# KeyuWu-CS/MonoHair

Hardware: AMD Instinct MI355X
Metric: PMVO iterations/sec (60x1080p views, 256^3 volume) (higher is better)
Workload: dtype f32

## Files before the change

### monohair_amd/csrc/pmvo_search.hip

```cpp
#include "mh_search_common.h"
#include "../../include/mh_pmvo_lab.h"

__device__ __forceinline__ void mh_sample_next(const float *__restrict__ cam, float X0, float X1, float X2,
                                               float ori_r, float ori_c, float Hf, float Wf, float off, float &S0,
                                               float &S1, float &S2, int forms) {
    alignas(16) float rec[16];
    mh_sample_rank(cam, X0, X1, X2, ori_r, ori_c, Hf, Wf, rec, forms);
    mh_sample_item(reinterpret_cast<const float4 *>(rec), off, S0, S1, S2);
}

__device__ __forceinline__ float mh_one_minus_abs(float x) {
    float r;
    asm("v_sub_f32_e64 %0, 1.0, |%1|" : "=v"(r) : "v"(x));
    return r;
}

template <int K, int T>
__global__ __launch_bounds__(T) void mh_search_kernel(MhViews vw, const float *__restrict__ offs, int S, int nrank,
                                                      int rank_step, const float *__restrict__ pts, int N, int P1,
                                                      float thr, const float *__restrict__ ori_c,
                                                      const int32_t *__restrict__ base_idx,
                                                      const float *__restrict__ base_val,
                                                      const float4 *__restrict__ taps, float *__restrict__ line_ori,
                                                      float *__restrict__ min_loss, uint8_t *__restrict__ high_conf,
                                                      float *__restrict__ best_sample, int32_t *__restrict__ best_rank,
                                                      int32_t *__restrict__ best_s, MhRule rule) {
    __shared__ float s_loss[MH_MAX_ITEMS];
    __shared__ uint8_t s_pos[MH_MAX_ITEMS];
    __shared__ float s_rl[MH_MAX_RANKS];
    __shared__ int s_ri[MH_MAX_RANKS];
    __shared__ int s_rh[MH_MAX_RANKS];

    const int n = blockIdx.x, tid = threadIdx.x;
    const int nitems = nrank * S;
    const int V = vw.V;
    const float Hf = (float)vw.H, Wf = (float)vw.W;
    const float P0 = pts[3 * n], P1x = pts[3 * n + 1], P2 = pts[3 * n + 2];

    float X0[K], X1[K], X2[K];
    MhCascV num[K], den[K];
    int cnt[K];
    const int tail_from = mh_tail_from(rule, n, S);
#pragma unroll
    for (int j = 0; j < K; ++j) {
        int it = j * T + tid;
        it = it < nitems ? it : 0;
        const int r = it / S, s = it - r * S;
        const int b = min(max(base_idx[(size_t)(r * rank_step) * N + n], 0), V - 1);
        const float2 oc = reinterpret_cast<const float2 *>(ori_c)[(size_t)b * N + n];
        mh_sample_next(vw.cams + b * MH_CAM_STRIDE, P0, P1x, P2, oc.x, oc.y, Hf, Wf, offs[s], X0[j], X1[j], X2[j],
                       mh_group_forms(rule, r, V, b, S));
        num[j] = den[j] = MhCascV{0.0f, 0.0f, 0.0f};
        cnt[j] = 0;
    }

    for (int v = 0; v < V; ++v) {
        if (v > 0 && (v & 15) == 0) {
#pragma unroll
            for (int j = 0; j < K; ++j) {
                mh_cascv_flush(num[j], v);
                mh_cascv_flush(den[j], v);
            }
        }
        const float4 *__restrict__ rec = taps + ((size_t)v * N + n) * P1;
        const float4 hdr = rec[0];
        if (hdr.y == -1.0f) continue;
        const int ntap = __float_as_int(hdr.x);
        const float *__restrict__ cam = vw.cams + v * MH_CAM_STRIDE;
        const float4 t0 = rec[1];
        {
            float dx[K], dy[K], ml[K], bc[K];
#pragma unroll
            for (int j = 0; j < K; ++j) {
                float row, col;
                mh_pixel_of(cam, X0[j], X1[j], X2[j], Hf, Wf, row, col);
                mh_unit2(row - hdr.z, col - hdr.w, dx[j], dy[j]);
                const float cs = t0.x * dx[j] + t0.y * dy[j];
                ml[j] = 1.0f - __builtin_fabsf(cs);
                bc[j] = t0.z;
            }
            for (int t = 1; t < ntap; ++t) {
                const float4 tp = rec[1 + t];
#pragma unroll
                for (int j = 0; j < K; ++j) {
                    const float cs = tp.x * dx[j] + tp.y * dy[j];
                    const float l = 1.0f - __builtin_fabsf(cs);
                    const bool upd = l < ml[j];
                    ml[j] = upd ? l : ml[j];
                    bc[j] = upd ? tp.z : bc[j];
                }
            }
#pragma unroll
            for (int j = 0; j < K; ++j) {
                const float w = bc[j];
                num[j].a0 = num[j].a0 + ml[j] * w;
                den[j].a0 = den[j].a0 + w;
                cnt[j] += (w > 0.0f) ? 1 : 0;
            }
        }
    }

#pragma unroll
    for (int j = 0; j < K; ++j) {
        const int it = j * T + tid;
        if (it < nitems) {
            float dn = mh_cascv_done(den[j]);
            float nm = mh_cascv_done(num[j]);
            int cn = cnt[j];
            if (it - (it / S) * S >= tail_from)
                mh_tail_item_sums(vw.cams, V, Hf, Wf, taps + (size_t)n * P1, (size_t)N * P1, nullptr, N, X0[j], X1[j], X2[j],
                                  nm, dn, cn);
            const float ratio = dn / (float)cn;
            s_pos[it] = (ratio > thr) ? 1 : 0;
            s_loss[it] = nm / dn;
        }
    }
    const bool all_nan = mh_point_pixel_not_finite(vw, P0, P1x, P2, N, tid, T);

    const int wave = tid >> 6, lane = tid & 63, nwaves = T >> 6;
    for (int r = wave; r < nrank; r += nwaves) {
        int npos = 0;
        for (int s0 = 0; s0 < S; s0 += MH_WAVE) {
            const int s = s0 + lane;
            npos += __popcll(__ballot(s < S && s_pos[r * S + s]));
        }
        const bool low = npos < 5;
        float bl = 0.0f;
        int bi = 0x7fffffff;
        for (int s = lane; s < S; s += MH_WAVE) {
            float l = all_nan ? __builtin_nanf("") : s_loss[r * S + s];
            if (!low && !s_pos[r * S + s]) l = 1.0f;
            if (bi == 0x7fffffff || mh_min_better(l, s, bl, bi)) {
                bl = l;
                bi = s;
            }
        }
#pragma unroll
        for (int o = 32; o > 0; o >>= 1) {
            const float ol = __shfl_xor(bl, o);
            const int oi = __shfl_xor(bi, o);
            if (oi != 0x7fffffff && (bi == 0x7fffffff || mh_min_better(ol, oi, bl, bi))) {
                bl = ol;
                bi = oi;
            }
        }
        if (lane == 0) {
            s_rl[r] = bl;
            s_ri[r] = bi;
            s_rh[r] = s_pos[r * S + bi];
        }
    }
    __syncthreads();

    if (tid == 0) {
        const float Hf = (float)vw.H, Wf = (float)vw.W;
        float ml = s_rl[0];
        int br = 0, bs = s_ri[0], hc = s_rh[0];
        for (int r = 1; r < nrank; ++r) {
            const float l = s_rl[r];
            if ((l < ml) && (base_val[(size_t)(r * rank_step) * N + n] > 0.0f)) {
                ml = l;
                br = r;
                bs = s_ri[r];
                hc = s_rh[r];
            }
        }
        const int b = min(max(base_idx[(size_t)(br * rank_step) * N + n], 0), V - 1);
        const float2 oc = reinterpret_cast<const float2 *>(ori_c)[(size_t)b * N + n];
        float B0, B1, B2;
        mh_sample_next(vw.cams + b * MH_CAM_STRIDE, P0, P1x, P2, oc.x, oc.y, Hf, Wf, offs[bs], B0, B1, B2,
                       mh_group_forms(rule, br, V, b, S));
        const float d0 = B0 - P0, d1 = B1 - P1x, d2 = B2 - P2;
        float s2 = d0 * d0;
        s2 = mh_fma(d1, d1, s2);
        s2 = mh_fma(d2, d2, s2);
        const float nrm = __builtin_sqrtf(s2);
        line_ori[3 * n] = d0 / nrm;
        line_ori[3 * n + 1] = d1 / nrm;
        line_ori[3 * n + 2] = d2 / nrm;
        min_loss[n] = ml;
        high_conf[n] = (uint8_t)hc;
        if (best_sample) {
            best_sample[3 * n] = B0;
            best_sample[3 * n + 1] = B1;
            best_sample[3 * n + 2] = B2;
        }
        if (best_rank) best_rank[n] = br;
        if (best_s) best_s[n] = bs;
    }
}

__device__ __forceinline__ float mh_vmul(float a, float b) {
    float r;
    asm("v_mul_f32_e32 %0, %1, %2" : "=v"(r) : "v"(a), "v"(b));
    return r;
}
__device__ __forceinline__ float mh_vadd(float a, float b) {
    float r;
    asm("v_add_f32_e32 %0, %1, %2" : "=v"(r) : "v"(a), "v"(b));
    return r;
}

template <int KA>
__device__ __forceinline__ void mh_tap_update(float (&ML)[KA], float (&BC)[KA], const float (&l)[KA], float cf) {
    if constexpr (KA == 4) {
        unsigned long long m0, m1, m2, m3;
        asm("v_cmp_lt_f32_e64 %[m0], %[l0], %[a0]\n\t"
            "v_cmp_lt_f32_e64 %[m1], %[l1], %[a1]\n\t"
            "v_cmp_lt_f32_e64 %[m2], %[l2], %[a2]\n\t"
            "v_cmp_lt_f32_e64 %[m3], %[l3], %[a3]\n\t"
            "v_cndmask_b32_e64 %[a0], %[a0], %[l0], %[m0]\n\t"
            "v_cndmask_b32_e64 %[a1], %[a1], %[l1], %[m1]\n\t"
            "v_cndmask_b32_e64 %[a2], %[a2], %[l2], %[m2]\n\t"
            "v_cndmask_b32_e64 %[a3], %[a3], %[l3], %[m3]\n\t"
            "v_cndmask_b32_e64 %[b0], %[b0], %[cf], %[m0]\n\t"
            "v_cndmask_b32_e64 %[b1], %[b1], %[cf], %[m1]\n\t"
            "v_cndmask_b32_e64 %[b2], %[b2], %[cf], %[m2]\n\t"
            "v_cndmask_b32_e64 %[b3], %[b3], %[cf], %[m3]"
            : [a0] "+v"(ML[0]), [a1] "+v"(ML[1]), [a2] "+v"(ML[2]), [a3] "+v"(ML[3]), [b0] "+v"(BC[0]),
              [b1] "+v"(BC[1]), [b2] "+v"(BC[2]), [b3] "+v"(BC[3]), [m0] "=&s"(m0), [m1] "=&s"(m1), [m2] "=&s"(m2),
              [m3] "=&s"(m3)
            : [l0] "v"(l[0]), [l1] "v"(l[1]), [l2] "v"(l[2]), [l3] "v"(l[3]), [cf] "v"(cf));
    } else if constexpr (KA == 3) {
        unsigned long long m0, m1, m2;
        asm("v_cmp_lt_f32_e64 %[m0], %[l0], %[a0]\n\t"
            "v_cmp_lt_f32_e64 %[m1], %[l1], %[a1]\n\t"
            "v_cmp_lt_f32_e64 %[m2], %[l2], %[a2]\n\t"
            "v_cndmask_b32_e64 %[a0], %[a0], %[l0], %[m0]\n\t"
            "v_cndmask_b32_e64 %[a1], %[a1], %[l1], %[m1]\n\t"
            "v_cndmask_b32_e64 %[a2], %[a2], %[l2], %[m2]\n\t"
            "v_cndmask_b32_e64 %[b0], %[b0], %[cf], %[m0]\n\t"
            "v_cndmask_b32_e64 %[b1], %[b1], %[cf], %[m1]\n\t"
            "v_cndmask_b32_e64 %[b2], %[b2], %[cf], %[m2]"
            : [a0] "+v"(ML[0]), [a1] "+v"(ML[1]), [a2] "+v"(ML[2]), [b0] "+v"(BC[0]), [b1] "+v"(BC[1]),
              [b2] "+v"(BC[2]), [m0] "=&s"(m0), [m1] "=&s"(m1), [m2] "=&s"(m2)
            : [l0] "v"(l[0]), [l1] "v"(l[1]), [l2] "v"(l[2]), [cf] "v"(cf));
    } else if constexpr (KA == 2) {
        unsigned long long m0, m1;
        asm("v_cmp_lt_f32_e64 %[m0], %[l0], %[a0]\n\t"
            "v_cmp_lt_f32_e64 %[m1], %[l1], %[a1]\n\t"
            "s_nop 0\n\t"
            "v_cndmask_b32_e64 %[a0], %[a0], %[l0], %[m0]\n\t"
            "v_cndmask_b32_e64 %[a1], %[a1], %[l1], %[m1]\n\t"
            "v_cndmask_b32_e64 %[b0], %[b0], %[cf], %[m0]\n\t"
            "v_cndmask_b32_e64 %[b1], %[b1], %[cf], %[m1]"
            : [a0] "+v"(ML[0]), [a1] "+v"(ML[1]), [b0] "+v"(BC[0]), [b1] "+v"(BC[1]), [m0] "=&s"(m0), [m1] "=&s"(m1)
            : [l0] "v"(l[0]), [l1] "v"(l[1]), [cf] "v"(cf));
    } else {
#pragma unroll
        for (int j = 0; j < KA; ++j) {
            const bool upd = l[j] < ML[j];
            ML[j] = upd ? l[j] : ML[j];
            BC[j] = upd ? cf : BC[j];
        }
    }
}

#define MH_KEY_C 1.00006103515625f
#define MH_KEY_E 6.103515625e-05f
#define MH_KEY_BAD 0xF0000000u
#ifndef MH_KEY_MIN_TAPS
#define MH_KEY_MIN_TAPS 10
#endif
#define MH_KEY_PAD 4
template <bool BIGP>
__device__ __forceinline__ int mh_key_walked(int c) {
    return (c - (BIGP ? 0 : 1) + MH_KEY_PAD - 1) & ~(MH_KEY_PAD - 1);
}
template <bool BIGP>
__device__ __forceinline__ int mh_key_staged(int c) {
    const int w = mh_key_walked<BIGP>(c);
    return w > c ? w : c;
}
__device__ unsigned long long mh_key_stats_dev[4];
extern "C" int mh_debug_key_stats(unsigned long long *out, int reset) {
    if (hipMemcpyFromSymbol(out, HIP_SYMBOL(mh_key_stats_dev), sizeof(unsigned long long) * 4) != hipSuccess) return -1;
    if (reset) {
        const unsigned long long z[4] = {0, 0, 0, 0};
        if (hipMemcpyToSymbol(HIP_SYMBOL(mh_key_stats_dev), z, sizeof(z)) != hipSuccess) return -1;
    }
    return 0;
}
#define MH_KEY_COUNT_ALWAYS(i) do { if ((tid & 63) == 0) atomicAdd(&mh_key_stats_dev[i], 1ull); } while (0)
#ifdef MH_KEY_STATS
#define MH_KEY_COUNT(i) MH_KEY_COUNT_ALWAYS(i)
#else
#define MH_KEY_COUNT(i) do { } while (0)
#endif
__device__ __forceinline__ unsigned mh_tap_key(float cs, int idx) {
    float t;
    unsigned k;
    asm("v_sub_f32_e64 %0, %2, |%1|" : "=v"(t) : "v"(cs), "s"(MH_KEY_C));
    asm("v_lshl_or_b32 %0, %1, 5, %2" : "=v"(k) : "v"(t), "s"(idx));
    return k;
}
__device__ __forceinline__ unsigned mh_min3u(unsigned a, unsigned b, unsigned c) {
    unsigned r;
    asm("v_min3_u32 %0, %1, %2, %3" : "=v"(r) : "v"(a), "v"(b), "v"(c));
    return r;
}

#include "mh_key_blocks.h"

#define MH_S3_GRP 4
#ifndef MH_S3_WAVES
#define MH_S3_WAVES 5
#endif
#ifndef MH_S3_WAVES_SELECT
#define MH_S3_WAVES_SELECT MH_S3_WAVES
#endif
#define MH_S3_CAP 1280

template <bool BIG>
struct MhCascS {
    float a0 = 0.0f, a1 = 0.0f, a2 = 0.0f;
    __device__ __forceinline__ void flush(int v) {
        a1 = a1 + a0;
        a0 = 0.0f;
        if constexpr (BIG) {
            if ((v & 0xF0) == 0) {
                a2 = a2 + a1;
                a1 = 0.0f;
            }
        }
    }
    __device__ __forceinline__ float done() const { return BIG ? (a0 + a1) + a2 : (a0 + a1); }
};

template <int KA, int T, bool BIGV, bool KEYS, bool BIGP>
__device__ __forceinline__ void mh_search_slices_lds(const MhViews &vw, const float *__restrict__ offs, int S,
                                                     int n, int N, int P1, float thr,
                                                     const float4 *__restrict__ taps, const uint8_t *__restrict__ vcnt,
                                                     int nact, int tid, float *s_loss, uint8_t *s_pos, float4 *s_taps,
                                                     const float4 *s_rank, int c_first) {
    constexpr int KN = KA > 0 ? KA : 1;
    constexpr int KM = KA;
    const int V = vw.V;
    const float Hf = (float)vw.H, Wf = (float)vw.W;
    float X0[KN], X1[KN], X2[KN];
    MhCascS<BIGV> num[KN], den[KN];
    int cnt[KN];
    if constexpr (KA > 0) {
        const unsigned inv = (1u << 20) / (unsigned)S + 1u;
#pragma unroll
        for (int j = 0; j < KA; ++j) {
            int it = j * T + tid;
            it = it < nact ? it : 0;
            const int r = (int)(((unsigned)it * inv) >> 20), s = it - r * S;
            mh_sample_item(s_rank + 4 * r, offs[s], X0[j], X1[j], X2[j]);
            num[j] = den[j] = MhCascS<BIGV>{};
            cnt[j] = 0;
        }
    }
    int nf = 16;
    auto flush_upto = [&](int v) {
        while (nf <= v) {
#pragma unroll
            for (int j = 0; j < KN; ++j) {
                num[j].flush(nf);
                den[j].flush(nf);
            }
            nf += 16;
        }
    };
    auto one_view = [&](int v, const float4 *rec, int ntap) {
        const float *__restrict__ cam = vw.cams + v * MH_CAM_STRIDE;
        const float4 hdr = rec[0];
        const float4 t0 = rec[1];
        float DX[KN], DY[KN], ML[KN], BC[KN];
#pragma unroll
        for (int jp = 0; jp < KA / 2; ++jp) {
            mh_v2f row, col, dx, dy;
            mh_pixel_of_fast2(cam, mh_v2f{X0[2 * jp], X0[2 * jp + 1]}, mh_v2f{X1[2 * jp], X1[2 * jp + 1]},
                              mh_v2f{X2[2 * jp], X2[2 * jp + 1]}, Hf, Wf, row, col);
            mh_unit2_fast2(row - mh_splat(hdr.z), col - mh_splat(hdr.w), dx, dy);
            DX[2 * jp] = dx.x;
            DX[2 * jp + 1] = dx.y;
            DY[2 * jp] = dy.x;
            DY[2 * jp + 1] = dy.y;
        }
        if constexpr (KA & 1) {
            mh_v2f row, col, dx, dy;
            mh_pixel_of_fast2(cam, mh_splat(X0[KA - 1]), mh_splat(X1[KA - 1]), mh_splat(X2[KA - 1]), Hf, Wf, row, col);
            mh_unit2_fast2(row - mh_splat(hdr.z), col - mh_splat(hdr.w), dx, dy);
            DX[KA - 1] = dx.x;
            DY[KA - 1] = dy.x;
        }
        constexpr int GRP = MH_S3_GRP;
        auto select_body = [&]() {
#pragma unroll
            for (int j = 0; j < KA; ++j) {
                ML[j] = mh_one_minus_abs(mh_vadd(mh_vmul(t0.x, DX[j]), mh_vmul(t0.y, DY[j])));
                BC[j] = t0.z;
            }
            auto process = [&](const float4 (&g)[GRP], int t) {
#pragma unroll
                for (int u = 0; u < GRP; ++u) {
                    if (t + u < ntap) {
                        const float4 tp = g[u];
                        float l[KN];
#pragma unroll
                        for (int j = 0; j < KA; ++j)
                            l[j] = mh_one_minus_abs(mh_vadd(mh_vmul(tp.x, DX[j]), mh_vmul(tp.y, DY[j])));
                        mh_tap_update<KN>(ML, BC, l, tp.z);
                    }
                }
            };
            float4 ga[GRP], gb[GRP];
#pragma unroll
            for (int u = 0; u < GRP; ++u) ga[u] = rec[2 + u];
            for (int t = 1; t < ntap;) {
#pragma unroll
                for (int u = 0; u < GRP; ++u) gb[u] = rec[1 + t + GRP + u];
                process(ga, t);
                t += GRP;
                if (t >= ntap) break;
#pragma unroll
                for (int u = 0; u < GRP; ++u) ga[u] = rec[1 + t + GRP + u];
                process(gb, t);
                t += GRP;
            }
        };
        __builtin_amdgcn_s_setprio(0);
        if constexpr (!KEYS) {
            select_body();
        } else {
            bool again = (ntap <= MH_KEY_MIN_TAPS) || !(t0.x == t0.x && t0.y == t0.y);
            MH_KEY_COUNT(0);
            if (again) MH_KEY_COUNT(1);
            if (!again) {
                const int ntp = mh_key_walked<BIGP>(ntap);
                unsigned ke[KN], ko[KN];
                const unsigned rec1 = (unsigned)(size_t)(const __attribute__((address_space(3))) float4 *)(rec + 1);
                auto process = [&](const float2 (&g)[GRP], int t) {
                    const int ib = (t & 63) >> 1;
                    static_assert(MH_KEY_PAD == 4 && GRP == 4, "the key block takes four taps");
                    if constexpr (KM > 0) mh_key_block4<KM, KN>(ke, ko, g, DX, DY, ib);
                };
                auto group = [&](int ta, int tb) {
                    const float2 *__restrict__ t2 = reinterpret_cast<const float2 *>(rec + 1);
                    float2 ga[GRP], gb[GRP];
#pragma unroll
                    for (int u = 0; u < GRP; ++u) ga[u] = t2[2 * (ta + u)];
                    if constexpr (BIGP || KM == 0) {
#pragma unroll
                        for (int j = 0; j < KN; ++j) ke[j] = ko[j] = 0xFFFFFFFFu;
                    } else {
                        const int is = ntap - 1;
                        const float2 ts = t2[2 * is];
                        const bool even = (is & 1) == 0;
#pragma unroll
                        for (int j = 0; j < KM; ++j) {
                            const unsigned k = mh_tap_key(mh_vadd(mh_vmul(ts.x, DX[j]), mh_vmul(ts.y, DY[j])), is >> 1);
                            ke[j] = even ? k : 0xFFFFFFFFu;
                            ko[j] = even ? 0xFFFFFFFFu : k;
                        }
                    }
                    for (int t = ta; t < tb;) {
#pragma unroll
                        for (int u = 0; u < GRP; ++u) gb[u] = t2[2 * (t + GRP + u)];
                        process(ga, t);
                        t += GRP;
                        if (t >= tb) break;
#pragma unroll
                        for (int u = 0; u < GRP; ++u) ga[u] = t2[2 * (t + GRP + u)];
                        process(gb, t);
                        t += GRP;
                    }
                };
                unsigned best[KN], badr[KN];
                auto winner = [&](int ta, bool first) {
#pragma unroll
                    for (int j = 0; j < KM; ++j) {
                        const bool odd = ko[j] < ke[j];
                        const unsigned kb = odd ? ko[j] : ke[j];
                        const unsigned ad = rec1 + 16u * (unsigned)ta + ((kb & 31u) << 5) + (odd ? 16u : 0u);
                        const bool take = first || kb < (best[j] & ~31u);
                        best[j] = take ? kb : best[j];
                        badr[j] = take ? ad : badr[j];
                    }
                };
                if constexpr (!BIGP) {
                    group(0, ntp);
                    winner(0, true);
                } else {
                    group(0, ntp < 64 ? ntp : 64);
                    winner(0, true);
                    for (int ta = 64; ta < ntp; ta += 64) {
                        group(ta, ntp < ta + 64 ? ntp : ta + 64);
                        winner(ta, false);
                    }
                }
                unsigned worst = best[0];
#pragma unroll
                for (int j = 1; j < KM; ++j) worst = max(worst, best[j]);
                const bool bad = worst >= MH_KEY_BAD;
#pragma unroll
                for (int j = 0; j < KM; ++j) {
                    BC[j] = *reinterpret_cast<const __attribute__((address_space(3))) float *>((size_t)(badr[j] + 8u));
                    ML[j] = __uint_as_float(__builtin_amdgcn_alignbit(7u, best[j], 5u)) - MH_KEY_E;
                }
                again = __ballot(bad) != 0ull;
                if (again) MH_KEY_COUNT_ALWAYS(2);
            }
            if (again) select_body();
        }
        __builtin_amdgcn_s_setprio(1);
#pragma unroll
        for (int j = 0; j < KA; ++j) {
            const float w = BC[j];
            num[j].a0 = num[j].a0 + ML[j] * w;
            den[j].a0 = den[j].a0 + w;
            cnt[j] += (w > 0.0f) ? 1 : 0;
        }
    };
    const int lane = tid & 63, wave = tid >> 6;
    for (int vb = 0; vb < V; vb += 64) {
        const int vv = vb + lane;
        const int c = vb == 0 ? c_first : ((vv < V) ? (int)vcnt[(size_t)vv * N + n] : 0);
        const int len = c ? ((KEYS && c > MH_KEY_MIN_TAPS) ? mh_key_staged<BIGP>(c) : c) + 1 : 0;
        int pre = len;
#pragma unroll
        for (int o = 1; o < 64; o <<= 1) {
            const int y = __shfl_up(pre, o);
            pre += (lane >= o) ? y : 0;
        }
        unsigned long long todo = __ballot(c != 0);
        int base = 0;
        while (todo) {
            const unsigned long long take = todo & __ballot(pre - base <= MH_S3_CAP);
            {
                unsigned long long m = take;
                int k = 0;
                while (m) {
                    const int b = (int)__builtin_ctzll(m);
                    m &= m - 1;
                    if ((k & (T / 64 - 1)) == wave) {
                        const int L = __builtin_amdgcn_readlane(len, b);
                        const int off = __builtin_amdgcn_readlane(pre, b) - L - base;
                        const float4 *__restrict__ src = taps + ((size_t)(vb + b) * N + n) * P1;
                        if constexpr (KEYS) {
                            const int lr = __builtin_amdgcn_readlane(c, b) + 1;
                            for (int i = lane; i < L; i += 64)
                                s_taps[off + i] = (i < lr) ? src[i] : make_float4(0.f, 0.f, 0.f, 0.f);
                        } else {
                            for (int i = lane; i < L; i += 64) s_taps[off + i] = src[i];
                        }
                    }
                    ++k;
                }
            }
            __syncthreads();
            if constexpr (KA > 0) {
                unsigned long long m = take;
                while (m) {
                    const int b = (int)__builtin_ctzll(m);
                    m &= m - 1;
                    flush_upto(vb + b);
                    const int L = __builtin_amdgcn_readlane(len, b);
                    const int off = __builtin_amdgcn_readlane(pre, b) - L - base;
                    one_view(vb + b, s_taps + off, KEYS ? __builtin_amdgcn_readlane(c, b) : L - 1);
                }
            }
            __syncthreads();
            base = __builtin_amdgcn_readlane(pre, 63 - (int)__builtin_clzll(take));
            todo &= ~take;
        }
    }
    if constexpr (KA > 0) {
        flush_upto(V - 1);
#pragma unroll
        for (int j = 0; j < KA; ++j) {
            const int it = j * T + tid;
            if (it < nact) {
                const float dn = den[j].done();
                const float nm = num[j].done();
                const float ratio = dn / (float)cnt[j];
                s_pos[it] = (ratio > thr) ? 1 : 0;
                s_loss[it] = nm / dn;
            }
        }
    }
}

template <int T, bool BIGV, bool KEYS, bool BIGP>
__global__ __launch_bounds__(T) __attribute__((amdgpu_waves_per_eu(KEYS ? MH_S3_WAVES : MH_S3_WAVES_SELECT))) void mh_search3_kernel(MhViews vw, const float *__restrict__ offs, int S, int nrank,
                                                       int rank_step, const float *__restrict__ pts, int N, int P1,
                                                       float thr, const float *__restrict__ ori_c,
                                                       const int32_t *__restrict__ base_idx,
                                                       const float *__restrict__ base_val,
                                                       const float4 *__restrict__ taps,
                                                       const uint8_t *__restrict__ vcnt,
                                                       const int32_t *__restrict__ order, float *__restrict__ line_ori,
                                                       float *__restrict__ min_loss, uint8_t *__restrict__ high_conf,
                                                       float *__restrict__ best_sample, int32_t *__restrict__ best_rank,
                                                       int32_t *__restrict__ best_s, MhRule rule) {
    __shared__ float4 s_taps[MH_S3_CAP + 8];
    __shared__ float s_loss[MH_MAX_ITEMS];
    __shared__ uint8_t s_pos[MH_MAX_ITEMS];
    __shared__ float s_rl[MH_MAX_RANKS];
    __shared__ int s_ri[MH_MAX_RANKS];
    __shared__ int s_rh[MH_MAX_RANKS];
    __shared__ float4 s_rank[MH_MAX_RANKS * 4];
    __shared__ float s_bval[MH_MAX_RANKS];
    __shared__ int s_tail;

    __builtin_amdgcn_s_setprio(1);
    const int tid = threadIdx.x;
    const int n = order ? order[blockIdx.x] : (int)blockIdx.x;
    const float P0 = pts[3 * n], P1x = pts[3 * n + 1], P2 = pts[3 * n + 2];
    const int c_first = ((tid & 63) < vw.V) ? (int)vcnt[(size_t)(tid & 63) * N + n] : 0;
    if (tid == 64) s_tail = mh_tail_from(rule, n, S);
    if (tid < nrank) {
        const size_t ro = (size_t)(tid * rank_step) * N + n;
        s_bval[tid] = base_val[ro];
        const int b = min(max(base_idx[ro], 0), vw.V - 1);
        const float2 oc = reinterpret_cast<const float2 *>(ori_c)[(size_t)b * N + n];
        mh_sample_rank(vw.cams + b * MH_CAM_STRIDE, P0, P1x, P2, oc.x, oc.y, (float)vw.H, (float)vw.W,
                       reinterpret_cast<float *>(s_rank + 4 * tid), mh_group_forms(rule, tid, vw.V, b, S));
    }
    __syncthreads();
    int nvalid = 1;
    for (int r = 1; r < nrank; ++r)
        if (s_bval[r] > 0.0f) nvalid = r + 1;
    const int nact = nvalid * S;
    const int wave0 = tid & ~63;
    int ka = 0;
    for (int j = 0; j < 4; ++j) ka += (j * T + wave0 < nact) ? 1 : 0;
#define MH_S3_ARGS vw, offs, S, n, N, P1, thr, taps, vcnt, nact, tid, s_loss, s_pos, s_taps, s_rank, c_first
    if (ka == 4) mh_search_slices_lds<4, T, BIGV, KEYS, BIGP>(MH_S3_ARGS);
    else if (ka == 3) mh_search_slices_lds<3, T, BIGV, KEYS, BIGP>(MH_S3_ARGS);
    else if (ka == 2) mh_search_slices_lds<2, T, BIGV, KEYS, BIGP>(MH_S3_ARGS);
    else if (ka == 1) mh_search_slices_lds<1, T, BIGV, KEYS, BIGP>(MH_S3_ARGS);
    else mh_search_slices_lds<0, T, BIGV, KEYS, BIGP>(MH_S3_ARGS);
#undef MH_S3_ARGS
    __syncthreads();
    if (s_tail < S) {
        const int tail_from = s_tail;
        for (int it = tid; it < nact; it += T) {
            const int r = it / S, s = it - r * S;
            if (s < tail_from) continue;
            float X0, X1, X2, nm, dn;
            int cnt;
            mh_sample_item(s_rank + 4 * r, offs[s], X0, X1, X2);
            mh_tail_item_sums(vw.cams, vw.V, (float)vw.H, (float)vw.W, taps + (size_t)n * P1, (size_t)N * P1, vcnt + n, N, X0, X1,
                              X2, nm, dn, cnt);
            s_pos[it] = (dn / (float)cnt > thr) ? 1 : 0;
            s_loss[it] = nm / dn;
        }
        __syncthreads();
    }

    const bool all_nan = mh_point_pixel_not_finite(vw, P0, P1x, P2, N, tid, T);
    const int wave = tid >> 6, lane = tid & 63, nwaves = T >> 6;
    for (int r = wave; r < nvalid; r += nwaves) {
        int npos = 0;
        for (int s0 = 0; s0 < S; s0 += MH_WAVE) {
            const int s = s0 + lane;
            npos += __popcll(__ballot(s < S && s_pos[r * S + s]));
        }
        const bool low = npos < 5;
        float bl = 0.0f;
        int bi = 0x7fffffff;
        for (int s = lane; s < S; s += MH_WAVE) {
            float l = all_nan ? __builtin_nanf("") : s_loss[r * S + s];
            if (!low && !s_pos[r * S + s]) l = 1.0f;
            if (bi == 0x7fffffff || mh_min_better(l, s, bl, bi)) {
                bl = l;
                bi = s;
            }
        }
#pragma unroll
        for (int o = 32; o > 0; o >>= 1) {
            const float ol = __shfl_xor(bl, o);
            const int oi = __shfl_xor(bi, o);
            if (oi != 0x7fffffff && (bi == 0x7fffffff || mh_min_better(ol, oi, bl, bi))) {
                bl = ol;
                bi = oi;
            }
        }
        if (lane == 0) {
            s_rl[r] = bl;
            s_ri[r] = bi;
            s_rh[r] = s_pos[r * S + bi];
        }
    }
    __syncthreads();

    if (tid == 0) {
        float ml = s_rl[0];
        int br = 0, bs = s_ri[0], hc = s_rh[0];
        for (int r = 1; r < nvalid; ++r) {
            const float l = s_rl[r];
            if ((l < ml) && (s_bval[r] > 0.0f)) {
                ml = l;
                br = r;
                bs = s_ri[r];
                hc = s_rh[r];
            }
        }
        float B0, B1, B2;
        mh_sample_item(s_rank + 4 * br, offs[bs], B0, B1, B2);
        const float d0 = B0 - P0, d1 = B1 - P1x, d2 = B2 - P2;
        float s2 = d0 * d0;
        s2 = mh_fma(d1, d1, s2);
        s2 = mh_fma(d2, d2, s2);
        const float nrm = __builtin_sqrtf(s2);
        line_ori[3 * n] = d0 / nrm;
        line_ori[3 * n + 1] = d1 / nrm;
        line_ori[3 * n + 2] = d2 / nrm;
        min_loss[n] = ml;
        high_conf[n] = (uint8_t)hc;
        if (best_sample) {
            best_sample[3 * n] = B0;
            best_sample[3 * n + 1] = B1;
            best_sample[3 * n + 2] = B2;
        }
        if (best_rank) best_rank[n] = br;
        if (best_s) best_s[n] = bs;
    }
}

__global__ __launch_bounds__(256) void mh_search_work_kernel(const uint8_t *__restrict__ cnt, int V, int N, int P1,
                                                             const float *__restrict__ base_val, int nrank,
                                                             int rank_step, int S, int T, int32_t *__restrict__ order,
                                                             int tail_n0) {
    const int wave = threadIdx.x >> 6, lane = threadIdx.x & 63;
    const int n = blockIdx.x * 4 + wave;
    if (n >= N) return;
    int nt = 0;
    for (int v = lane; v < V; v += MH_WAVE) nt += cnt[(size_t)v * N + n];
#pragma unroll
    for (int o = 32; o > 0; o >>= 1) nt += __shfl_xor(nt, o);
    const bool usable = lane > 0 && lane < nrank && base_val[(size_t)(lane * rank_step) * N + n] > 0.0f;
    const unsigned long long m = __ballot(usable);
    const int nvalid = m ? (64 - __builtin_clzll(m)) : 1;
    if (lane == 0) order[n] = n >= tail_n0 ? 0 : mh_work_class(nt, nvalid, V, P1, S, T);
}

__global__ __launch_bounds__(256) void mh_group_sizes_kernel(const int32_t *__restrict__ base_idx, int N, int V,
                                                             int rank_step, int32_t *__restrict__ gcnt) {
    extern __shared__ int s_g[];
    const int r = blockIdx.y, tid = threadIdx.x;
    for (int i = tid; i < V; i += 256) s_g[i] = 0;
    __syncthreads();
    const int n = blockIdx.x * 256 + tid;
    if (n < N) {
        const int b = base_idx[(size_t)(r * rank_step) * N + n];
        if (b >= 0 && b < V) atomicAdd(&s_g[b], 1);
    }
    __syncthreads();
    for (int i = tid; i < V; i += 256)
        if (s_g[i]) atomicAdd(&gcnt[(((int)blockIdx.x & (MH_GROUP_COPIES - 1)) * MH_GROUP_RANKS + r) * V + i], s_g[i]);
}

__global__ __launch_bounds__(1024) void mh_search_order_kernel(int N, int32_t *__restrict__ order) {
    __shared__ int s_hist[MH_ORDER_BUCKETS];
    __shared__ int s_part[1024 / 64];
    const int tid = threadIdx.x;
    s_hist[tid] = 0;
    __syncthreads();
    for (int n = tid; n < N; n += 1024) atomicAdd(&s_hist[order[n]], 1);
    __syncthreads();
    const int mine = s_hist[tid];
    int incl = mine;
#pragma unroll
    for (int o = 1; o < 64; o <<= 1) {
        const int x = __shfl_up(incl, o);
        if ((tid & 63) >= o) incl += x;
    }
    if ((tid & 63) == 63) s_part[tid >> 6] = incl;
    __syncthreads();
    int base = 0;
    for (int w = 0; w < (tid >> 6); ++w) base += s_part[w];
    __syncthreads();
    s_hist[tid] = base + incl - mine;
    __syncthreads();
    for (int n = tid; n < N; n += 1024) order[N + atomicAdd(&s_hist[order[n]], 1)] = n;
}

extern "C" int mh_launch_search(MhViews vw, const float *offs, int S, int nrank, int rank_step, const float *pts,
                                int N, int P1, float thr, const float *ori_c, const int32_t *base_idx,
                                const float *base_val, const float4 *taps, int32_t *order ,
                                const uint8_t *cnt ,
                                float *line_ori, float *min_loss, uint8_t *high_conf, float *best_sample,
                                int32_t *best_rank, int32_t *best_s, MhSearchPlan plan, int rule_mode, int fma_min_cols,
                                int sum_block, int32_t *gcnt ,
                                int groups_ready ,
                                hipStream_t st) {
    const int nitems = nrank * S;
    if (nitems > MH_MAX_ITEMS || nrank > MH_MAX_RANKS || nitems < 1) return -1;
    if (sum_block < 0) return -1;
    MhRule rule;
    rule.mode = rule_mode;
    rule.fma_min_cols = fma_min_cols;
    rule.gcnt = (rule_mode == 0) ? gcnt : nullptr;
    if (rule_mode == 0 && !gcnt) return -1;
    const long long cols = (long long)N * S;
    rule.tail_col0 = sum_block ? cols - cols % sum_block : cols;
    const bool portable = plan.portable || !cnt;
    if (rule.gcnt && !groups_ready && plan.part != MhSearchPlan::PART_KERNEL_ONLY) {
        if (hipMemsetAsync(gcnt, 0, sizeof(int32_t) * (size_t)MH_GROUP_COPIES * MH_GROUP_RANKS * vw.V, st) != hipSuccess) return -1;
        hipLaunchKernelGGL(mh_group_sizes_kernel, dim3((N + 255) / 256, nrank), dim3(256), sizeof(int) * (size_t)vw.V, st,
                           base_idx, N, vw.V, rank_step, gcnt);
    }
    if (!portable) {
        const int32_t *ord = nullptr;
        if (plan.order != MhSearchPlan::ORDER_NATURAL && order && N > 1) {
            if (plan.part != MhSearchPlan::PART_KERNEL_ONLY) {
                if (plan.order == MhSearchPlan::ORDER_BY_WORK)
                    hipLaunchKernelGGL(mh_search_work_kernel, dim3((N + 3) / 4), dim3(256), 0, st, cnt, vw.V, N, P1, base_val,
                                       nrank, rank_step, S, 256, order, (int)(rule.tail_col0 / S));
                hipLaunchKernelGGL(mh_search_order_kernel, dim3(1), dim3(1024), 0, st, N, order);
            }
            ord = order + N;
        }
        if (plan.part == MhSearchPlan::PART_PRE_ONLY) return (int)hipGetLastError();
#define MH_S3_LAUNCH(BIG, KEYS, BIGP)                                                                                   \
    hipLaunchKernelGGL((mh_search3_kernel<256, BIG, KEYS, BIGP>), dim3(N), dim3(256), 0, st, vw, offs, S, nrank, rank_step, \
                       pts, N, P1, thr, ori_c, base_idx, base_val, taps, cnt, ord, line_ori, min_loss, high_conf,       \
                       best_sample, best_rank, best_s, rule)
        const bool bigp = P1 - 1 > 64;
        if (vw.V > 256) {
            if (plan.select_body) MH_S3_LAUNCH(true, false, false);
            else if (bigp) MH_S3_LAUNCH(true, true, true);
            else MH_S3_LAUNCH(true, true, false);
        } else {
            if (plan.select_body) MH_S3_LAUNCH(false, false, false);
            else if (bigp) MH_S3_LAUNCH(false, true, true);
            else MH_S3_LAUNCH(false, true, false);
        }
#undef MH_S3_LAUNCH
    } else {
        hipLaunchKernelGGL((mh_search_kernel<4, 256>), dim3(N), dim3(256), 0, st, vw, offs, S, nrank, rank_step, pts, N, P1,
                           thr, ori_c, base_idx, base_val, taps, line_ori, min_loss, high_conf, best_sample, best_rank,
                           best_s, rule);
    }
    return (int)hipGetLastError();
}

extern "C" int mh_preload_pmvo_search() {
    hipFuncAttributes a;
    return (int)hipFuncGetAttributes(&a, reinterpret_cast<const void *>(&mh_search_order_kernel));
}
```

Before: 1690.

## Stage first tap batch via async global_load_lds overlapping rank setup

```diff
diff --git a/monohair_amd/csrc/pmvo_search.hip b/monohair_amd/csrc/pmvo_search.hip
--- a/monohair_amd/csrc/pmvo_search.hip
+++ b/monohair_amd/csrc/pmvo_search.hip
@@ -327,12 +327,55 @@
     __device__ __forceinline__ float done() const { return BIG ? (a0 + a1) + a2 : (a0 + a1); }
 };
 
+__device__ __forceinline__ int mh_wave_prefix_sum(int x) {
+#define MH_DPP_ADD(CTRL, ROWS) x += __builtin_amdgcn_update_dpp(0, x, CTRL, ROWS, 0xF, false)
+    MH_DPP_ADD(0x111, 0xF);
+    MH_DPP_ADD(0x112, 0xF);
+    MH_DPP_ADD(0x114, 0xF);
+    MH_DPP_ADD(0x118, 0xF);
+    MH_DPP_ADD(0x142, 0xA);
+    MH_DPP_ADD(0x143, 0xC);
+#undef MH_DPP_ADD
+    return x;
+}
+
+__device__ const float4 mh_zero_tap = {0.0f, 0.0f, 0.0f, 0.0f};
+__device__ __forceinline__ void mh_stage_list(const float4 *__restrict__ src, float4 *dst, int nrec, int nfill, int lane) {
+    for (int i0 = 0; i0 < nfill; i0 += 64) {
+        const int i = i0 + lane;
+        if (i < nfill) {
+            const float4 *g = (i < nrec) ? src + i : &mh_zero_tap;
+            __builtin_amdgcn_global_load_lds((const __attribute__((address_space(1))) void *)g,
+                                             (__attribute__((address_space(3))) void *)(dst + i0), 16, 0, 0);
+        }
+    }
+}
+
+template <bool KEYS, bool BIGP>
+__device__ __forceinline__ int mh_list_records(int c) {
+    return c ? ((KEYS && c > MH_KEY_MIN_TAPS) ? mh_key_staged<BIGP>(c) : c) + 1 : 0;
+}
+template <int T, bool KEYS>
+__device__ __forceinline__ void mh_stage_batch(const float4 *__restrict__ taps, float4 *s_taps, int vb, int n, int N, int P1,
+                                               int c, int len, int pre, int base, unsigned long long take, int lane, int wave) {
+    const unsigned place = __builtin_amdgcn_mbcnt_hi((unsigned)(take >> 32), __builtin_amdgcn_mbcnt_lo((unsigned)take, 0u));
+    unsigned long long m = take & __ballot((int)(place & (T / 64 - 1)) == wave);
+    while (m) {
+        const int b = (int)__builtin_ctzll(m);
+        m &= m - 1;
+        const int L = __builtin_amdgcn_readlane(len, b);
+        const int off = __builtin_amdgcn_readlane(pre, b) - L - base;
+        const int lr = KEYS ? __builtin_amdgcn_readlane(c, b) + 1 : L;
+        mh_stage_list(taps + ((size_t)(vb + b) * N + n) * P1, s_taps + off, lr, L, lane);
+    }
+}
+
 template <int KA, int T, bool BIGV, bool KEYS, bool BIGP>
 __device__ __forceinline__ void mh_search_slices_lds(const MhViews &vw, const float *__restrict__ offs, int S,
                                                      int n, int N, int P1, float thr,
                                                      const float4 *__restrict__ taps, const uint8_t *__restrict__ vcnt,
                                                      int nact, int tid, float *s_loss, uint8_t *s_pos, float4 *s_taps,
-                                                     const float4 *s_rank, int c_first) {
+                                                     const float4 *s_rank, int c_first, int pre_first) {
     constexpr int KN = KA > 0 ? KA : 1;
     constexpr int KM = KA;
     const int V = vw.V;
@@ -514,43 +557,22 @@
             cnt[j] += (w > 0.0f) ? 1 : 0;
         }
     };
-    const int lane = tid & 63, wave = tid >> 6;
+    const int lane = tid & 63, wave = __builtin_amdgcn_readfirstlane(tid >> 6);
     for (int vb = 0; vb < V; vb += 64) {
         const int vv = vb + lane;
         const int c = vb == 0 ? c_first : ((vv < V) ? (int)vcnt[(size_t)vv * N + n] : 0);
-        const int len = c ? ((KEYS && c > MH_KEY_MIN_TAPS) ? mh_key_staged<BIGP>(c) : c) + 1 : 0;
-        int pre = len;
-#pragma unroll
-        for (int o = 1; o < 64; o <<= 1) {
-            const int y = __shfl_up(pre, o);
-            pre += (lane >= o) ? y : 0;
-        }
+        const int len = mh_list_records<KEYS, BIGP>(c);
+        const int pre = vb == 0 ? pre_first : mh_wave_prefix_sum(len);
+        bool staged = vb == 0;
         unsigned long long todo = __ballot(c != 0);
         int base = 0;
         while (todo) {
             const unsigned long long take = todo & __ballot(pre - base <= MH_S3_CAP);
-            {
-                unsigned long long m = take;
-                int k = 0;
-                while (m) {
-                    const int b = (int)__builtin_ctzll(m);
-                    m &= m - 1;
-                    if ((k & (T / 64 - 1)) == wave) {
-                        const int L = __builtin_amdgcn_readlane(len, b);
-                        const int off = __builtin_amdgcn_readlane(pre, b) - L - base;
-                        const float4 *__restrict__ src = taps + ((size_t)(vb + b) * N + n) * P1;
-                        if constexpr (KEYS) {
-                            const int lr = __builtin_amdgcn_readlane(c, b) + 1;
-                            for (int i = lane; i < L; i += 64)
-                                s_taps[off + i] = (i < lr) ? src[i] : make_float4(0.f, 0.f, 0.f, 0.f);
-                        } else {
-                            for (int i = lane; i < L; i += 64) s_taps[off + i] = src[i];
-                        }
-                    }
-                    ++k;
-                }
-            }
-            __syncthreads();
+            if (!staged) {
+                mh_stage_batch<T, KEYS>(taps, s_taps, vb, n, N, P1, c, len, pre, base, take, lane, wave);
+                __syncthreads();
+            }
+            staged = false;
             if constexpr (KA > 0) {
                 unsigned long long m = take;
                 while (m) {
@@ -610,6 +632,11 @@
     const int n = order ? order[blockIdx.x] : (int)blockIdx.x;
     const float P0 = pts[3 * n], P1x = pts[3 * n + 1], P2 = pts[3 * n + 2];
     const int c_first = ((tid & 63) < vw.V) ? (int)vcnt[(size_t)(tid & 63) * N + n] : 0;
+    const int len_first = mh_list_records<KEYS, BIGP>(c_first);
+    const int pre_first = mh_wave_prefix_sum(len_first);
+    mh_stage_batch<T, KEYS>(taps, s_taps, 0, n, N, P1, c_first, len_first, pre_first, 0,
+                            __ballot(c_first != 0) & __ballot(pre_first <= MH_S3_CAP), tid & 63,
+                            __builtin_amdgcn_readfirstlane(tid >> 6));
     if (tid == 64) s_tail = mh_tail_from(rule, n, S);
     if (tid < nrank) {
         const size_t ro = (size_t)(tid * rank_step) * N + n;
@@ -627,7 +654,7 @@
     const int wave0 = tid & ~63;
     int ka = 0;
     for (int j = 0; j < 4; ++j) ka += (j * T + wave0 < nact) ? 1 : 0;
-#define MH_S3_ARGS vw, offs, S, n, N, P1, thr, taps, vcnt, nact, tid, s_loss, s_pos, s_taps, s_rank, c_first
+#define MH_S3_ARGS vw, offs, S, n, N, P1, thr, taps, vcnt, nact, tid, s_loss, s_pos, s_taps, s_rank, c_first, pre_first
     if (ka == 4) mh_search_slices_lds<4, T, BIGV, KEYS, BIGP>(MH_S3_ARGS);
     else if (ka == 3) mh_search_slices_lds<3, T, BIGV, KEYS, BIGP>(MH_S3_ARGS);
     else if (ka == 2) mh_search_slices_lds<2, T, BIGV, KEYS, BIGP>(MH_S3_ARGS);
```

New measurement: 1712 (median of 6 runs). +1.3%, better.
